# ROBOT-WSC/RGC-SLAM

Measured on AMD Instinct MI355X. Metric: registered scans/sec (16-beam -> 1M-pt map), higher is better.
Workload: dtype f32 points and neighbour search, f64 covariances and solve

## Files before the change

rgc-slam_amd/csrc/rgc_api.hip:

```cpp
#include "rgc_ctx.h"

static std::mutex g_live_mutex;
static std::unordered_set<const rgc_ctx*> g_live;
static std::atomic<unsigned long long> g_next_uid{1};

namespace rgcapi {

constexpr int kMaxK = 32;
constexpr unsigned kDevEvent = hipEventDisableTiming | hipEventReleaseToDevice;

bool ctx_alive(const rgc_ctx* c) {
  std::lock_guard<std::mutex> lk(g_live_mutex);
  return g_live.count(c) != 0;
}

int fail(rgc_ctx* c, int code, const char* fmt, ...) {
  if (c) {
    va_list ap;
    va_start(ap, fmt);
    vsnprintf(c->err, sizeof(c->err), fmt, ap);
    va_end(ap);
  }
  return code;
}
// ... 24 lines not shown
  memset(&at, 0, sizeof(at));
  if (hipPointerGetAttributes(&at, p) != hipSuccess) {
    (void)hipGetLastError();
    return fail(c, RGC_ERR_INVALID, "%s: %p is not memory the HIP runtime knows (a host pointer passed as a device pointer?)", what, p);
  }
  if (at.type != hipMemoryTypeDevice) return fail(c, RGC_ERR_INVALID, "%s: %p is not device memory", what, p);
  if (at.device != c->device) return fail(c, RGC_ERR_INVALID, "%s: %p lives on device %d, the context on device %d", what, p, at.device, c->device);
  void* base = nullptr;
  size_t size = 0;
  if (hipMemGetAddressRange((hipDeviceptr_t*)&base, &size, (hipDeviceptr_t)const_cast<void*>(p)) != hipSuccess) { (void)hipGetLastError(); return RGC_OK; }
  const size_t off = (size_t)((const char*)p - (const char*)base);
  if (off + bytes > size) return fail(c, RGC_ERR_INVALID, "%s: %zu bytes asked of an allocation that has %zu behind %p", what, bytes, size - off, p);
  return RGC_OK;
}

static void release(DevBuf& b) {
  if (b.p && !b.borrowed) (void)hipFree(b.p);
  b.p = nullptr;
  b.cap = 0;
  b.borrowed = false;
}

static void release_cloud(Cloud& cl) {
  for (DevBuf* b : {&cl.in_copy, &cl.cell_of, &cl.slot_of, &cl.cnt, &cl.start, &cl.block_sums, &cl.order_tmp, &cl.P, &cl.nx, &cl.ny, &cl.nz, &cl.segs,
                    &cl.cell_voxel, &cl.vox, &cl.vox_cell, &cl.need, &cl.qlist, &cl.cell_list, &cl.seed, &cl.nbr, &cl.rank_of, &cl.pos_of, &cl.qrank,
                    &cl.map_copy, &cl.todo, &cl.cache_small, &cl.c6})
    release(*b);
}

namespace {
struct ProfScope {
  rgc_ctx* c;
  bool on;
  ProfRegion r{};
  hipStream_t st;
  ProfScope(rgc_ctx* ctx, int kind, long long points, hipStream_t stream = nullptr) : c(ctx), on(ctx->prof_on && ((ctx->prof_mask >> kind) & 1u)), st(stream ? stream : ctx->stream) {
    if (!on) return;
    auto get = [&](hipEvent_t* e) {
      if (!c->ev_pool.empty()) { *e = c->ev_pool.back(); c->ev_pool.pop_back(); return true; }
      return hipEventCreate(e) == hipSuccess;
    };
    if (!get(&r.a)) { on = false; return; }
// ... 245 lines not shown
        if ((rc = ensure(c, cl.cnt, sizeof(int) * wc1 + 256))) return rc;
        if ((rc = ensure(c, cl.start, sizeof(int) * wc1))) return rc;
        if ((rc = ensure(c, cl.block_sums, sizeof(long long) * (wc1 / 2048 + 2)))) return rc;
        if (is_target && (rc = ensure(c, cl.cell_voxel, sizeof(int) * (size_t)w.ncell))) return rc;
        if (is_target) {
          const size_t vw = (size_t)(n < w.ncell ? n : w.ncell);
          if ((rc = ensure(c, cl.vox, sizeof(double) * rgck::kVoxRec * vw))) return rc;
          if ((rc = ensure(c, cl.vox_cell, sizeof(int) * vw))) return rc;
        }
      }
    }
    cl.grid = g;
    const size_t nc1 = (size_t)g.ncell + 1;
    const size_t ntot = nc1;
    int rc;
    if ((rc = ensure(c, cl.cell_of, sizeof(int) * n))) return rc;
    if ((rc = ensure(c, cl.slot_of, sizeof(int) * n))) return rc;
    size_t want_cells = ntot;
    if (hint && hint->reach_xy > 0) {
      const double e = hint->reach_xy / res + 6.0, ez = hint->reach_z / res + 6.0;
      const double cells = e * e * ez * 1.05;
      if (cells < 2.0e9 && cells <= (double)c->prm.max_cells && (size_t)cells > want_cells) want_cells = (size_t)cells;
    }
    if ((rc = ensure(c, cl.cnt, sizeof(int) * std::max(ntot, want_cells) + 256))) return rc;
    if ((rc = ensure(c, cl.start, sizeof(int) * std::max(nc1, want_cells)))) return rc;
    if ((rc = ensure(c, cl.block_sums, sizeof(long long) * (std::max(ntot, want_cells) / 2048 + 2)))) return rc;
    if ((rc = ensure(c, cl.order_tmp, sizeof(long long) * n))) return rc;
    if ((rc = ensure(c, cl.P, sizeof(float4) * ((size_t)n + 4)))) return rc;
    if ((rc = ensure(c, cl.segs, rgck::deferred_bytes(n)))) return rc;
    if ((rc = ensure(c, cl.nx, sizeof(double) * n))) return rc;
    if ((rc = ensure(c, cl.ny, sizeof(double) * n))) return rc;
    if ((rc = ensure(c, cl.nz, sizeof(double) * n))) return rc;
    if (is_target && (rc = ensure(c, cl.cell_voxel, sizeof(int) * std::max((size_t)g.ncell, want_cells)))) return rc;
    if (cl.cnt.p != cl.cnt_seen) { cl.cnt_clean = 0; cl.cnt_seen = cl.cnt.p; }
    if (cl.cnt_clean < ntot) {
      const size_t fill = std::min(cl.cnt.cap, (sizeof(int) * ntot + 255) & ~(size_t)255);
      HIPCHK(c, hipMemsetAsync(cl.cnt.p, 0, fill, s));
      cl.cnt_clean = fill / sizeof(int);
    }
    rgck::count_cells(s, cl.in, cl.stride_f, n, g, (int*)cl.cell_of.p, (int*)cl.slot_of.p, (int*)cl.cnt.p, hi, spec ? dsm + 6 : nullptr,
                      fuse_reframe ? &cl.rf : nullptr);
    rgck::scan_cells(s, (int*)cl.cnt.p, (int*)cl.start.p, (int)ntot, cl.block_sums.p, is_target ? (int*)cl.cell_voxel.p : nullptr,
                     is_target ? c->d_small + 7 : nullptr, hi, is_target ? nullptr : (float*)(c->d_small + 23));
    const bool with_cache = is_target && &cl == &c->tgt && cl.cache_on;
    const rgck::KnnSeeds sd = cloud_seeds(cl, is_target);
    rgck::place(s, n, (const int*)cl.cell_of.p, (const int*)cl.slot_of.p, (const int*)cl.start.p, (unsigned long long*)cl.order_tmp.p, hi,
                with_cache ? &sd.cache : nullptr);
    rgck::rank_gather(s, cl.in, cl.stride_f, n, (const int*)cl.cell_of.p, (const int*)cl.start.p, (const unsigned long long*)cl.order_tmp.p,
                      (float4*)cl.P.p, (int*)cl.segs.p, hi, with_cache ? &sd.cache : nullptr);
  }
  cl.lazy = 0;
  if (is_target && &cl == &c->tgt && c->lazy_margin > 0 && !c->lm_host && !general_route(c) && map_wide_r_of(c, cl) == 0) {
    int rc;
    const size_t vmax = (size_t)(n < cl.grid.ncell ? n : cl.grid.ncell);
    if ((rc = ensure(c, cl.vox, sizeof(double) * rgck::kVoxRec * vmax))) return rc;
    if ((rc = ensure(c, cl.vox_cell, sizeof(int) * vmax))) return rc;
    cl.lazy = 1;
    cl.nvox = -1;
    HIPCHK(c, hipGetLastError());
    HIPCHK(c, hipEventRecord(c->tgt_prepared, s));
    cl.ready = true;
    return RGC_OK;
  }
  cl.prepared_recorded = false;
// ... 299 lines not shown

int check_target_owner(rgc_ctx* c) {
  if (!c->tgt_owner) return RGC_OK;
  bool alive;
  unsigned long long owner_gen = 0;
  {
    std::lock_guard<std::mutex> lk(g_live_mutex);
    alive = g_live.count(c->tgt_owner) != 0 && c->tgt_owner->uid == c->tgt_owner_uid;
    if (alive) owner_gen = c->tgt_owner->tgt_generation;
  }
  if (!alive) {
    c->tgt_owner = nullptr;
    for (DevBuf* b : {&c->tgt.in_copy, &c->tgt.cell_of, &c->tgt.slot_of, &c->tgt.cnt, &c->tgt.start, &c->tgt.block_sums, &c->tgt.order_tmp, &c->tgt.P,
                      &c->tgt.nx, &c->tgt.ny, &c->tgt.nz, &c->tgt.segs, &c->tgt.cell_voxel, &c->tgt.vox, &c->tgt.vox_cell, &c->tgt.c6})
      release(*b);
    c->tgt.ready = false;
    c->tgt.n = 0;
    return fail(c, RGC_ERR_NO_INPUT, "the context whose target this one shared has been destroyed");
  }
  if (owner_gen != c->tgt_owner_gen)
    return fail(c, RGC_ERR_INVALID, "the shared target was rebuilt by its owner: rgc_share_target again");
  return RGC_OK;
}

static int validate_clouds(rgc_ctx* c, bool whole_target = true) {
  if (solve_in_flight(c)) return fail(c, RGC_ERR_INVALID, "a solve is in flight on this context: call rgc_align_end first");
  { int rc = check_target_owner(c); if (rc) return rc; }
  if ((c->tgt.ready && c->tgt.spec_used) || (c->src.ready && c->src.spec_used)) {
    HIPCHK(c, hipStreamSynchronize(c->stream2));
    HIPCHK(c, hipMemcpyAsync(c->h_small + 6, c->d_small + 6, sizeof(int), hipMemcpyDeviceToHost, c->stream));
// ... 160 lines not shown
  rgck::bbox(s, cl.in, cl.stride_f, n, cell, dsm, dsm + 6);
  HIPCHK(c, hipMemcpyAsync(hsm, dsm, words * sizeof(int), hipMemcpyDeviceToHost, s));
  HIPCHK(c, hipStreamSynchronize(s));
  if (hsm[6]) return fail(c, RGC_ERR_NONFINITE, "%s contains non-finite or absurd coordinates", name);
  int minc[3], dim[3];
  double ncell = 1.0;
  for (int a = 0; a < 3; a++) {
    minc[a] = hsm[a];
    dim[a] = hsm[3 + a] - hsm[a] + 1;
    ncell *= (double)dim[a];
  }
  if (ncell > (double)c->prm.max_cells || ncell > 2.0e9) return fail(c, RGC_ERR_GRID_TOO_LARGE, "%s exceeds max_cells", grid_name);
  const rgck::Grid g = rgck::make_grid(minc, dim, cell);
  cl.grid = g;
  const size_t nc1 = (size_t)g.ncell + 1;
  if ((rc = ensure(c, cl.cell_of, sizeof(int) * n))) return rc;
  if ((rc = ensure(c, cl.slot_of, sizeof(int) * n))) return rc;
  if ((rc = ensure(c, cl.cnt, sizeof(int) * nc1 + 256))) return rc;
  if ((rc = ensure(c, cl.start, sizeof(int) * nc1))) return rc;
  if (with_voxels && (rc = ensure(c, cl.cell_voxel, sizeof(int) * nc1))) return rc;
  if ((rc = ensure(c, cl.block_sums, sizeof(long long) * (nc1 / 2048 + 2)))) return rc;
  if ((rc = ensure(c, cl.order_tmp, sizeof(long long) * n))) return rc;
  if ((rc = ensure(c, cl.P, sizeof(float4) * ((size_t)n + 4)))) return rc;
  HIPCHK(c, hipMemsetAsync(cl.cnt.p, 0, (sizeof(int) * nc1 + 255) & ~(size_t)255, s));
  rgck::count_cells(s, cl.in, cl.stride_f, n, g, (int*)cl.cell_of.p, (int*)cl.slot_of.p, (int*)cl.cnt.p);
  rgck::scan_cells(s, (int*)cl.cnt.p, (int*)cl.start.p, (int)nc1, cl.block_sums.p, with_voxels ? (int*)cl.cell_voxel.p : nullptr, with_voxels ? dsm + 7 : nullptr);
  rgck::place(s, n, (const int*)cl.cell_of.p, (const int*)cl.slot_of.p, (const int*)cl.start.p, (unsigned long long*)cl.order_tmp.p);
  rgck::rank_gather(s, cl.in, cl.stride_f, n, (const int*)cl.cell_of.p, (const int*)cl.start.p, (const unsigned long long*)cl.order_tmp.p, (float4*)cl.P.p);
  return RGC_OK;
}

}

using namespace rgcapi;

extern "C" {

void rgc_default_params(rgc_params* p) {
  if (!p) return;
  p->voxel_res = 1.0;
  p->max_iterations = 25;
  p->lm_max_iterations = 10;
  p->rotation_eps = 2e-3;
// ... 188 lines not shown
  if ((rc = fetch_nvox(owner))) return fail(c, rc, "rgc_share_target: %s", owner->err);
  HIPCHK(c, hipStreamSynchronize(owner->stream2));
  HIPCHK(c, hipStreamSynchronize(owner->stream));
  HIPCHK(c, hipStreamSynchronize(c->stream2));
  HIPCHK(c, hipStreamSynchronize(c->stream));
  Cloud& d = c->tgt;
  const Cloud& o = owner->tgt;
  release_cloud(d);
  DevBuf* db[] = {&d.in_copy, &d.cell_of, &d.slot_of, &d.cnt, &d.start, &d.block_sums, &d.order_tmp, &d.P, &d.nx, &d.ny, &d.nz, &d.segs,
                  &d.cell_voxel, &d.vox, &d.vox_cell, &d.c6};
  const DevBuf* ob[] = {&o.in_copy, &o.cell_of, &o.slot_of, &o.cnt, &o.start, &o.block_sums, &o.order_tmp, &o.P, &o.nx, &o.ny, &o.nz, &o.segs,
                        &o.cell_voxel, &o.vox, &o.vox_cell, &o.c6};
  d.general = o.general;
  for (size_t k = 0; k < sizeof(db) / sizeof(db[0]); k++) { db[k]->p = ob[k]->p; db[k]->cap = ob[k]->cap; db[k]->borrowed = ob[k]->p != nullptr; }
  d.in = o.in; d.stride_f = o.stride_f; d.n = o.n; d.grid = o.grid; d.grid = o.grid; d.nvox = o.nvox; d.deferred_seen = o.deferred_seen;
  d.spec_ok = false; d.spec_used = false; d.cnt_clean = 0; d.cnt_seen = nullptr; d.lazy = 0;
  d.ready = true;
  const int small[2] = {0, o.nvox};
  HIPCHK(c, hipMemcpyAsync(c->d_small + 6, small, sizeof(small), hipMemcpyHostToDevice, c->stream));
  HIPCHK(c, hipStreamSynchronize(c->stream));
  c->tgt_owner = owner;
  c->tgt_owner_gen = owner->tgt_generation;
  c->tgt_owner_uid = owner->uid;
  c->map_bound = false;
  c->corr_valid = c->gicp_valid = false;
  c->deferred_known = false;
  c->main_has_target_prep = false;
  c->stats.n_target = o.n; c->stats.target_cells = o.grid.ncell; c->stats.n_voxels = o.nvox;
  return RGC_OK;
}

// ... 746 lines not shown
```

rgc-slam_amd/csrc/rgc_api_pre.hip:

```cpp
#include "rgc_ctx.h"

using namespace rgcapi;

int rgcapi::stage_in(rgc_ctx* c, const float* p, int n, int stride_bytes, int on_device, const float** d_in) {
  if (n > (1 << 27)) return fail(c, RGC_ERR_INVALID, "cloud has %d points, the limit is 2^27", n);
  if (on_device) {
    if (n > 0) { const int rk = check_device_range(c, p, (size_t)n * stride_bytes - (stride_bytes - 12), "input cloud"); if (rk) return rk; }
    *d_in = p;
    return RGC_OK;
  }
  const size_t bytes = (size_t)n * stride_bytes;
  int rc = ensure(c, c->pre_in, bytes);
  if (rc) return rc;
  HIPCHK(c, hipMemcpyAsync(c->pre_in.p, p, bytes, hipMemcpyHostToDevice, c->stream));
  *d_in = (const float*)c->pre_in.p;
  return RGC_OK;
}

extern "C" {

int rgc_deskew(rgc_ctx* c, float* xyzi, int n, int stride_bytes, const double q[4], const double t[3], int on_device) {
  if (!c || !xyzi || !q || !t || n < 0) return RGC_ERR_INVALID;
  if (stride_bytes < 16 || (stride_bytes & 3) || stride_bytes > 4096) return fail(c, RGC_ERR_INVALID, "de-skew needs x,y,z,intensity: stride_bytes >= 16");
  if (n == 0) return RGC_OK;
// ... 208 lines not shown
      seg_shift = 3;
      while (seg_shift < 30 && (double)(((long long)g.div[0] + (1ll << seg_shift) - 1) >> seg_shift) > nseg_max) seg_shift++;
    }
  }
  const size_t nr1 = (size_t)g.div[1] * (size_t)g.div[2] * (size_t)rgck::vg_segments(g, seg_shift) + 1;
  if ((rc = ensure(c, cl.cell_of, sizeof(int) * n))) return rc;
  if ((rc = ensure(c, cl.slot_of, sizeof(int) * n))) return rc;
  if ((rc = ensure(c, c->vg_pos, sizeof(int) * n))) return rc;
  if ((rc = ensure(c, c->vg_order, sizeof(int) * n))) return rc;
  if ((rc = ensure(c, c->vg_tmp, sizeof(long long) * n))) return rc;
  if ((rc = ensure(c, c->vg_leaf, sizeof(long long) * n))) return rc;
  if ((rc = ensure(c, cl.cnt, sizeof(int) * nr1))) return rc;
  if ((rc = ensure(c, cl.start, sizeof(int) * nr1))) return rc;
  const size_t row_bs = sizeof(long long) * (nr1 / 2048 + 2);
  if ((rc = ensure(c, cl.block_sums, row_bs + sizeof(int) * ((size_t)n / 2048 + 2)))) return rc;
  if (cl.cnt.p != cl.cnt_seen) { cl.cnt_clean = 0; cl.cnt_seen = cl.cnt.p; }
  if (cl.cnt_clean < nr1) {
    const size_t fill = std::min(cl.cnt.cap, (sizeof(int) * nr1 + 255) & ~(size_t)255);
    HIPCHK(c, hipMemsetAsync(cl.cnt.p, 0, fill, s));
  }
  cl.cnt_clean = std::max(cl.cnt_clean, nr1);
  if (!c->vg_flags_clean) HIPCHK(c, hipMemsetAsync(dsm + 6, 0, sizeof(int), s));
  c->vg_flags_clean = false;
  const bool packed = rgck::vg_rows(s, d_in, stride_f, n, inv, g, edge, seg_shift, (int*)cl.cell_of.p, (int*)cl.slot_of.p, (int*)c->vg_pos.p, (int*)cl.cnt.p,
                                    (int*)cl.start.p, cl.block_sums.p, (unsigned long long*)c->vg_tmp.p, (int*)c->vg_order.p, (unsigned long long*)c->vg_leaf.p,
                                    (int*)((char*)cl.block_sums.p + row_bs), d_out, dsm + 5);
  rt->chain = 1; rt->leaf_buckets = dense ? 1 : 0; rt->seg_shift = seg_shift; rt->nseg = rgck::vg_segments(g, seg_shift); rt->packed = packed ? 1 : 0;
  rt->edge = edge; rt->flags = 0;
  for (int a = 0; a < 3; a++) { rt->minb[a] = g.minb[a]; rt->div[a] = g.div[a]; }
  if (h_result) {
// ... 383 lines not shown
```

rgc-slam_amd/csrc/rgc_ctx.h:

```cpp
#pragma once
#include "../../include/rgc_hip.h"

#include <hip/hip_runtime.h>

#include <cfloat>
#include <climits>
#include <cmath>
#include <cstdarg>
#include <cstdint>
#include <cstdio>
#include <cstdlib>
#include <cstring>
#include <atomic>
#include <chrono>
#include <mutex>
#include <new>
#include <unordered_map>
#include <unordered_set>
#include <vector>

#include "rgc_kernels.h"

namespace rgcapi {

// ... 49 lines not shown
  bool ready = false;
  bool covs_user = false;
  DevBuf in_copy, cell_of, slot_of, cnt, start, block_sums, order_tmp, P, nx, ny, nz;
  DevBuf c6;
  bool general = false;
  DevBuf segs;
  int deferred_seen = -1;
  rgck::Grid grid{};
  rgck::Grid spec_grid{};
  bool spec_ok = false;
  bool spec_used = false;
  bool reframe_pending = false;
  rgck::Reframe rf{};
  size_t cnt_clean = 0;
  const void* cnt_seen = nullptr;
  DevBuf cell_voxel, vox, vox_cell;
  int nvox = -1;
  int lazy = 0;
  DevBuf need, qlist, cell_list;
  int need_stamp = 0;
  const void* need_seen = nullptr;
  int lazy_nq_seen = -1, lazy_ncell_seen = -1;
  DevBuf seed;
  const void* seed_key = nullptr;
  int seed_n = 0;
  bool seed_on = false;
  bool seed_warm = false;
  float seed_slack = 0.f;
  DevBuf nbr, rank_of, pos_of, qrank, map_copy, todo, cache_small;
  bool cache_on = false;
// ... 174 lines not shown
    if (_e != hipSuccess) {                                                                                \
      (void)hipGetLastError();              \
      return rgcapi::fail((c), RGC_ERR_HIP, "%s failed: %s (%s:%d)", #expr, hipGetErrorString(_e), __FILE__, __LINE__);               \
    }                                                                                                      \
  } while (0)

int fail(rgc_ctx* c, int code, const char* fmt, ...);
int ensure(rgc_ctx* c, DevBuf& b, size_t bytes);
int check_device_range(rgc_ctx* c, const void* p, size_t bytes, const char* what);
bool ctx_alive(const rgc_ctx* c);
const rgc_ctx::BoxHint* find_hint(const rgc_ctx* c, const void* p, int n);
void put_hint(rgc_ctx* c, const void* p, int n, const double lo[3], const double hi[3], double reach_xy = 0, double reach_z = 0);
void hint_from_leaf_grid(rgc_ctx* c, const float* out , int n_out, const rgck::LeafGrid& g, float leaf);
bool map_prep_finished(rgc_ctx* c);
int set_cloud(rgc_ctx* c, Cloud& cl, bool is_target, const float* xyz, int n, int stride_bytes, bool on_device, const rgck::Reframe* rf = nullptr);
int build_measured_grid(rgc_ctx* c, Cloud& cl, double cell, int* dsm, int* hsm, bool with_voxels, const char* name, const char* grid_name);
rgck::Pose pose_from(const double T[16]);
rgck::PoseF posef_from(const float T[16]);
int check_target_owner(rgc_ctx* c);
int need_inputs(rgc_ctx* c, bool validate = true);
int do_fitness(rgc_ctx* c, const float T[16], double* out);
void unpack_system(const double sums[28], double H[36], double b[6]);

inline bool solve_in_flight(const rgc_ctx* c) { return c->pend.active || c->gen_res.on; }
inline bool stride_ok(int stride_bytes) { return stride_bytes >= 12 && !(stride_bytes & 3) && stride_bytes <= 4096; }
template <class T>
inline bool pose12_finite(const T* m) {
  for (int i = 0; i < 12; i++)
    if (!std::isfinite(m[i])) return false;
  return true;
// ... 30 lines not shown
```

rgc-slam_amd/csrc/rgc_kernels.h:

```cpp
#pragma once
#include <hip/hip_runtime.h>

#include <cmath>

namespace rgck {

struct Grid {
  int minc[3];
  int dim[3];
  double res;
  int ncell;
  double inv_res;
};
inline double grid_inv_res(double res) {
  int e;
  return std::frexp(res, &e) == 0.5 ? 1.0 / res : 0.0;
}
inline Grid make_grid(const int minc[3], const int dim[3], double res) {
  Grid g{};
  double nc = 1.0;
  for (int a = 0; a < 3; a++) { g.minc[a] = minc[a]; g.dim[a] = dim[a]; nc *= (double)dim[a]; }
  g.res = res;
  g.inv_res = grid_inv_res(res);
  g.ncell = nc <= 2.0e9 ? (int)nc : -1;
// ... 38 lines not shown
  double fit_sum;
  int nvox, def_t, def_s, pad;
  int gen, cmd, mode, cur;
  float src_sq; int pad2;
  int lazy_nq, lazy_ncell;
};
struct LmInit { double x0[16], rot_eps, trans_eps, init_factor; int max_outer, max_inner; };
struct LmEarly { double x0[16]; int pad, pad2, outer, gen; };
struct FeParams { int n_scans; double min_range, max_range; };
struct LeafGrid { int minb[3]; int div[3]; };

constexpr int kAccum = 28;
constexpr int kVoxRec = 10;

void bbox(hipStream_t s, const float* in, int stride_f, int n, double res, int* mm6, int* flags, int hi = 0);
void count_cells(hipStream_t s, const float* in, int stride_f, int n, Grid g, int* cell_of, int* slot_of, int* cnt, int hi = 0, int* guard = nullptr,
                 const Reframe* rf = nullptr);
void scan_cells(hipStream_t s, int* cnt, int* start, int n, void* block_sums, int* cell_voxel, int* nvox, int hi = 0,
                float* sum_sq = nullptr );
void place(hipStream_t s, int n, const int* cell_of, const int* slot_of, const int* start, unsigned long long* order_tmp, int hi = 0,
           const KnnCache* cache = nullptr );
void exclusive_scan(hipStream_t s, const int* in, int* out, int n, int* block_sums , int hi = 0);
void rank_gather(hipStream_t s, const float* in, int stride_f, int n, const int* cell_of, const int* start,
                 const unsigned long long* order_tmp, float4* P, int* zero_me = nullptr, int hi = 0, const KnnCache* cache = nullptr);
size_t deferred_bytes(int n);
struct KnnSeeds {
  float* seed = nullptr;
  float slack = 0.f;
  bool warm = false;
  KnnCache cache;
};
bool knn_seeds_apply(int n, int k);
void knn_bulk(hipStream_t s, bool is_target, const float4* P, const int* start, Grid g, int n, int k, const void* deferred, double* nx,
              double* ny, double* nz, const int* guard = nullptr, int wide_r = 0,
              hipEvent_t ev0 = nullptr, hipEvent_t ev1 = nullptr ,
              const int* qlist = nullptr, const int* nq = nullptr, int q_est = 0, const KnnSeeds& seeds = KnnSeeds{},
              int stream_coop_waves = 0);
constexpr int kDeferredSlotEmptyByte = 0x80;
void footprint(hipStream_t s, const float* in, int stride_f, int n, Pose T, Grid g, int* need, int stamp, int margin, const float4* P, int n_map,
// ... 118 lines not shown
```

rgc-slam_amd/csrc/rgc_kernels.hip:

```cpp
#include "rgc_kernels.h"
#include "rgc_nn.h"
#include "rgc_lm.h"
#include <hip/hip_ext.h>

#include <limits.h>
#include <stddef.h>

#include <type_traits>

namespace rgck {

constexpr int WAVE = 64;

__device__ __forceinline__ int voxel_coord1(float x, double res) { return (int)floor((double)x / res - 0.5); }

__device__ __forceinline__ int wave_min(int v) {
#pragma unroll
  for (int o = 32; o > 0; o >>= 1) v = min(v, __shfl_xor(v, o));
  return v;
}
__device__ __forceinline__ int wave_max(int v) {
#pragma unroll
  for (int o = 32; o > 0; o >>= 1) v = max(v, __shfl_xor(v, o));
  return v;
// ... 128 lines not shown
}

__device__ __forceinline__ constexpr int row_dy(int r, int D, int R) { return r % D - R; }
__device__ __forceinline__ constexpr int row_dz(int r, int D, int R) { return r / D - R; }

__device__ __forceinline__ float4 reframe_point(const Reframe& rf, int i) {
  const float* p = rf.src + (size_t)i * rf.src_stride_f;
  const Quat& q = rf.q;
  const double vx = (double)p[0], vy = (double)p[1], vz = (double)p[2];
  double ux = q.y * vz - q.z * vy, uy = q.z * vx - q.x * vz, uz = q.x * vy - q.y * vx;
  ux += ux; uy += uy; uz += uz;
  return make_float4((float)(vx + q.w * ux + (q.y * uz - q.z * uy) + rf.t[0]), (float)(vy + q.w * uy + (q.z * ux - q.x * uz) + rf.t[1]),
                     (float)(vz + q.w * uz + (q.x * uy - q.y * ux) + rf.t[2]), rf.src_stride_f > 3 ? p[3] : 0.f);
}

template <bool kReframe>
__global__ void k_count(const float* __restrict__ in, int stride_f, int n, Grid g, int* __restrict__ cell_of, int* __restrict__ slot_of,
                        int* cnt, int* guard, int prio, Reframe rf) {
  wave_prio(prio);
  const int i = blockIdx.x * blockDim.x + threadIdx.x;
  const bool valid = i < n;
  const int lane = threadIdx.x & (WAVE - 1);
  int c = -1 - lane;
#ifdef RGC_LAB_TURN
  if (kReframe && i == 0) {
    const unsigned long long now = wall_clock64(), post = atomicExch(&g_lab_turn[3], 0ull);
    if (post) { atomicAdd(&g_lab_turn[0], now - post); atomicAdd(&g_lab_turn[1], 1ull); atomicMax(&g_lab_turn[2], now - post); }
  }
#endif
  if (valid) {
    float pt[3];
    if (kReframe) {
      if (rf.copy) {
// ... 16 lines not shown
    int cx, cy, cz;
    if (guard) {
      const float x = p[0], y = p[1], z = p[2];
      const bool fin = fabsf(x) <= 1.0e8f && fabsf(y) <= 1.0e8f && fabsf(z) <= 1.0e8f;
      cx = fin ? cell_coord(x, g) - g.minc[0] : 0;
      cy = fin ? cell_coord(y, g) - g.minc[1] : 0;
      cz = fin ? cell_coord(z, g) - g.minc[2] : 0;
      const bool inside = cx >= 0 && cx < g.dim[0] && cy >= 0 && cy < g.dim[1] && cz >= 0 && cz < g.dim[2];
      if (!fin || !inside) { atomicOr(guard, fin ? 2 : 1); cx = cy = cz = 0; }
    } else {
      cx = cell_coord(p[0], g) - g.minc[0];
      cy = cell_coord(p[1], g) - g.minc[1];
      cz = cell_coord(p[2], g) - g.minc[2];
    }
    c = cell_index(g, cx, cy, cz);
    cell_of[i] = c;
  }
  unsigned long long todo = __ballot(valid);
  int lead = lane, rank = 0, group = 1;
  while (todo) {
    const int l0 = __ffsll((long long)todo) - 1;
    const int cl = __shfl(c, l0);
    const unsigned long long same = __ballot(valid && c == cl);
    if (valid && c == cl) {
      lead = l0;
      rank = __popcll(same & ((1ull << lane) - 1ull));
      group = __popcll(same);
    }
    todo &= ~same;
  }
  int base = 0;
  if (valid && lane == lead) base = atomicAdd(&cnt[c], group);
  base = __shfl(base, lead);
  if (valid) slot_of[i] = base + rank;
}

constexpr int SCAN_T = 256, SCAN_V = 8, SCAN_B = SCAN_T * SCAN_V;

__device__ __forceinline__ int block_exclusive_scan(int v, int* total) {
  __shared__ int wsum[SCAN_T / WAVE];
  int lane = threadIdx.x & (WAVE - 1), w = threadIdx.x / WAVE;
  int inc = v;
#pragma unroll
  for (int o = 1; o < WAVE; o <<= 1) {
    int t = __shfl_up(inc, o);
    if (lane >= o) inc += t;
  }
  if (lane == WAVE - 1) wsum[w] = inc;
  __syncthreads();
  int base = 0, tot = 0;
#pragma unroll
  for (int j = 0; j < SCAN_T / WAVE; j++) {
// ... 197 lines not shown
#pragma unroll
  for (int j = 0; j < SCAN_V; j++) {
    const int i = base + j;
    if (i < n) {
      start[i] = (int)(unsigned)ex;
      if (cell_voxel && i < n - 1) cell_voxel[i] = v[j] > 0 ? (int)(ex >> 32) : -1;
    }
    ex += scan_value(v[j]);
  }
}

constexpr int kOrdIdxBits = 27, kOrdCntBits = 18;
constexpr unsigned long long kOrdIdxMask = (1ull << kOrdIdxBits) - 1ull;
constexpr int kOrdCntMax = (1 << kOrdCntBits) - 1;
__device__ __forceinline__ bool cache_redo(const KnnCache& kc) { return *kc.epoch == kc.frame || kc.overflow[(kc.frame - 1) & 1] == kc.frame - 1; }
__global__ void k_place(int n, const int* __restrict__ cell_of, const int* __restrict__ slot_of, const int* __restrict__ start,
                        unsigned long long* __restrict__ order_tmp, int prio, KnnCache kc) {
  wave_prio(prio);
  const int i = blockIdx.x * blockDim.x + threadIdx.x;
  if (kc.nbr && i < kTodoLists && cache_redo(kc)) kc.todo_cnt[i] = 0;
  if (i >= n) return;
  const int c = cell_of[i], slot = slot_of[i];
  const int s0 = start[c], cnt = start[c + 1] - s0;
  const bool big = cnt > kOrdCntMax;
  order_tmp[s0 + slot] = (unsigned long long)(unsigned)i | ((unsigned long long)(big ? 0 : slot) << kOrdIdxBits) |
                         ((unsigned long long)(big ? 0 : cnt) << (kOrdIdxBits + kOrdCntBits));
}

__global__ void k_rank_gather(const float* __restrict__ in, int stride_f, int n, const int* __restrict__ cell_of,
                              const int* __restrict__ start, const unsigned long long* __restrict__ order_tmp, float4* __restrict__ P, int* zero_me,
                              int prio, KnnCache kc) {
  wave_prio(prio);
  int s = blockIdx.x * blockDim.x + threadIdx.x;
  if (s == 0 && zero_me) { zero_me[0] = 0; zero_me[1] = 0; zero_me[2] = 0; }
  if (s < 4) P[n + s] = make_float4(1.0e30f, 1.0e30f, 1.0e30f, __int_as_float(-1));
  if (s >= n) return;
  const unsigned long long rec = order_tmp[s];
  const int i = (int)(rec & kOrdIdxMask);
  const bool ranked = kc.nbr && !cache_redo(kc);
  int my_rank = 0;
  if (ranked) my_rank = kc.rank_of[i];
  const int cnt = (int)(rec >> (kOrdIdxBits + kOrdCntBits)) & kOrdCntMax;
  int s0, s1;
  if (cnt > 0) {
    s0 = s - ((int)(rec >> kOrdIdxBits) & kOrdCntMax);
    s1 = s0 + cnt;
  } else {
    const int c = cell_of[i];
    s0 = start[c];
    s1 = start[c + 1];
  }
  const float* p = in + (size_t)i * stride_f;
  const float px = p[0], py = p[1], pz = p[2];
  const unsigned* lo = reinterpret_cast<const unsigned*>(order_tmp);
  constexpr unsigned kLoMask = (unsigned)kOrdIdxMask;
  int rank = 0;
  int t = s0;
  for (; t + 8 <= s1; t += 8) {
    unsigned o[8];
#pragma unroll
    for (int u = 0; u < 8; u++) o[u] = lo[2 * (size_t)(t + u)];
#pragma unroll
    for (int u = 0; u < 8; u++) rank += ((int)(o[u] & kLoMask) < i);
// ... 3007 lines not shown
                  int want_H, double* partials, double* out56) {
  MapregPose ps[2];
  for (int b = 0; b < 2; b++) {
    const double* q = x14 + 7 * b;
    ps[b] = MapregPose{feat[2 * b], fac[2 * b], nfeat[2 * b], feat[2 * b + 1], fac[2 * b + 1], nfeat[2 * b + 1], Quat{q[0], q[1], q[2], q[3]},
                       {q[4], q[5], q[6]}};
  }
  const int nb = max(max(mapreg_blocks(nfeat[0], nfeat[1]), mapreg_blocks(nfeat[2], nfeat[3])), 1);
  hipLaunchKernelGGL(k_mapreg_terms, dim3(nb, 2), dim3(LIN_T), 0, s, ps[0], ps[1], huber_a, want_H, partials);
  hipLaunchKernelGGL(k_mapreg_fold, dim3(2 * kAccum), dim3(WAVE), 0, s, partials, nb, out56);
}

void bbox(hipStream_t s, const float* in, int stride_f, int n, double res, int* mm6, int* flags, int hi) {
  hipLaunchKernelGGL(k_bbox, dim3(min(nblk(n, 256), 1024)), dim3(256), 0, s, in, stride_f, n, res, mm6, flags, hi);
}
void count_cells(hipStream_t s, const float* in, int stride_f, int n, Grid g, int* cell_of, int* slot_of, int* cnt, int hi, int* guard,
                 const Reframe* rf) {
  if (rf) hipLaunchKernelGGL(k_count<true>, dim3(nblk(n, kGridT)), dim3(kGridT), 0, s, in, 4, n, g, cell_of, slot_of, cnt, guard, hi, *rf);
  else hipLaunchKernelGGL(k_count<false>, dim3(nblk(n, kGridT)), dim3(kGridT), 0, s, in, stride_f, n, g, cell_of, slot_of, cnt, guard, hi, Reframe{});
}
void scan_cells(hipStream_t s, int* cnt, int* start, int n, void* block_sums, int* cell_voxel, int* nvox, int hi, float* sum_sq) {
  const int nb = nblk(n, SCAN_B);
  unsigned long long* bs = (unsigned long long*)block_sums;
  if (nb > 1 || sum_sq) hipLaunchKernelGGL(k_cells_reduce, dim3(nb), dim3(SCAN_T), 0, s, cnt, n, bs, hi, sum_sq);
  if (nb <= 4096) {
    hipLaunchKernelGGL(k_cells_scan_write<true>, dim3(nb), dim3(SCAN_T), 0, s, cnt, start, n, bs, nb, cell_voxel, nvox, hi);
  } else {
    hipLaunchKernelGGL(k_cells_scan_sums, dim3(1), dim3(SCAN_T), 0, s, bs, nb, nvox, hi);
    hipLaunchKernelGGL(k_cells_scan_write<false>, dim3(nb), dim3(SCAN_T), 0, s, cnt, start, n, bs, nb, cell_voxel, nvox, hi);
  }
}
void place(hipStream_t s, int n, const int* cell_of, const int* slot_of, const int* start, unsigned long long* order_tmp, int hi, const KnnCache* cache) {
  hipLaunchKernelGGL(k_place, dim3(nblk(n, kGridT)), dim3(kGridT), 0, s, n, cell_of, slot_of, start, order_tmp, hi, cache ? *cache : KnnCache{});
}
void exclusive_scan(hipStream_t s, const int* in, int* out, int n, int* block_sums, int hi) {
  const int nb = nblk(n, SCAN_B);
  hipLaunchKernelGGL(k_scan_block, dim3(nb), dim3(SCAN_T), 0, s, in, out, n, block_sums, hi);
  if (nb > 1) {
    hipLaunchKernelGGL(k_scan_sums, dim3(1), dim3(SCAN_T), 0, s, block_sums, nb, hi);
    hipLaunchKernelGGL(k_scan_add, dim3(nb), dim3(SCAN_T), 0, s, out, n, block_sums, hi);
  }
}
void rank_gather(hipStream_t s, const float* in, int stride_f, int n, const int* cell_of, const int* start,
                 const unsigned long long* order_tmp, float4* P, int* zero_me, int hi, const KnnCache* cache) {
  hipLaunchKernelGGL(k_rank_gather, dim3(nblk(n, kGridT)), dim3(kGridT), 0, s, in, stride_f, n, cell_of, start, order_tmp, P, zero_me, hi,
                     cache ? *cache : KnnCache{});
}
size_t deferred_bytes(int n) { return sizeof(int) * (2 * (size_t)n + 16); }

static Deferred deferred_of(const void* buf, int n) {
  int* base = (int*)const_cast<void*>(buf);
  return Deferred{base + 16, (float*)(base + 16 + (size_t)n), base, nullptr, nullptr, nullptr, nullptr, 0.f, KnnCache{}, 0,
                  0, base + 1, reinterpret_cast<unsigned long long*>(base + 16), 0};
}

template <int KC, bool kExact>
static void knn_bulk_kc(hipStream_t s, bool is_target, const float4* P, const int* start, Grid g, int n, int k, const void* deferred,
                        double* nx, double* ny, double* nz, const int* guard, int wide_r, hipEvent_t ev0, hipEvent_t ev1,
                        const int* qlist, const int* nq, int q_est, const KnnSeeds& seeds, int stream_coop_waves) {
  Deferred df = deferred_of(deferred, n);
  df.guard = guard;
// ... 188 lines not shown
```

Before: 2744.

## Fuse per-block cell totals into count kernel and pack cell/slot as int2

```diff
diff --git a/rgc-slam_amd/csrc/rgc_api.hip b/rgc-slam_amd/csrc/rgc_api.hip
--- a/rgc-slam_amd/csrc/rgc_api.hip
+++ b/rgc-slam_amd/csrc/rgc_api.hip
@@ -62,6 +62,17 @@
   return RGC_OK;
 }
 
+int ensure_block_sums(rgc_ctx* c, Cloud& cl, size_t bytes, hipStream_t s) {
+  int rc;
+  if ((rc = ensure(c, cl.block_sums, bytes))) return rc;
+  if (cl.block_sums.p != cl.bs_seen || cl.block_sums.cap != cl.bs_cap) {
+    HIPCHK(c, hipMemsetAsync(cl.block_sums.p, 0, cl.block_sums.cap, s));
+    cl.bs_seen = cl.block_sums.p;
+    cl.bs_cap = cl.block_sums.cap;
+  }
+  return RGC_OK;
+}
+
 static void release(DevBuf& b) {
   if (b.p && !b.borrowed) (void)hipFree(b.p);
   b.p = nullptr;
@@ -74,6 +85,7 @@
                     &cl.cell_voxel, &cl.vox, &cl.vox_cell, &cl.need, &cl.qlist, &cl.cell_list, &cl.seed, &cl.nbr, &cl.rank_of, &cl.pos_of, &cl.qrank,
                     &cl.map_copy, &cl.todo, &cl.cache_small, &cl.c6})
     release(*b);
+  cl.bs_seen = nullptr;
 }
 
 namespace {
@@ -349,8 +361,7 @@
     const size_t nc1 = (size_t)g.ncell + 1;
     const size_t ntot = nc1;
     int rc;
-    if ((rc = ensure(c, cl.cell_of, sizeof(int) * n))) return rc;
-    if ((rc = ensure(c, cl.slot_of, sizeof(int) * n))) return rc;
+    if ((rc = ensure(c, cl.cell_of, sizeof(int2) * n))) return rc;
     size_t want_cells = ntot;
     if (hint && hint->reach_xy > 0) {
       const double e = hint->reach_xy / res + 6.0, ez = hint->reach_z / res + 6.0;
@@ -359,7 +370,7 @@
     }
     if ((rc = ensure(c, cl.cnt, sizeof(int) * std::max(ntot, want_cells) + 256))) return rc;
     if ((rc = ensure(c, cl.start, sizeof(int) * std::max(nc1, want_cells)))) return rc;
-    if ((rc = ensure(c, cl.block_sums, sizeof(long long) * (std::max(ntot, want_cells) / 2048 + 2)))) return rc;
+    if ((rc = ensure_block_sums(c, cl, sizeof(long long) * (std::max(ntot, want_cells) / 2048 + 2), s))) return rc;
     if ((rc = ensure(c, cl.order_tmp, sizeof(long long) * n))) return rc;
     if ((rc = ensure(c, cl.P, sizeof(float4) * ((size_t)n + 4)))) return rc;
     if ((rc = ensure(c, cl.segs, rgck::deferred_bytes(n)))) return rc;
@@ -373,16 +384,15 @@
       HIPCHK(c, hipMemsetAsync(cl.cnt.p, 0, fill, s));
       cl.cnt_clean = fill / sizeof(int);
     }
-    rgck::count_cells(s, cl.in, cl.stride_f, n, g, (int*)cl.cell_of.p, (int*)cl.slot_of.p, (int*)cl.cnt.p, hi, spec ? dsm + 6 : nullptr,
-                      fuse_reframe ? &cl.rf : nullptr);
+    rgck::count_cells(s, cl.in, cl.stride_f, n, g, (int2*)cl.cell_of.p, (int*)cl.cnt.p, is_target ? cl.block_sums.p : nullptr, hi,
+                      spec ? dsm + 6 : nullptr, fuse_reframe ? &cl.rf : nullptr);
     rgck::scan_cells(s, (int*)cl.cnt.p, (int*)cl.start.p, (int)ntot, cl.block_sums.p, is_target ? (int*)cl.cell_voxel.p : nullptr,
-                     is_target ? c->d_small + 7 : nullptr, hi, is_target ? nullptr : (float*)(c->d_small + 23));
+                     is_target ? c->d_small + 7 : nullptr, hi, is_target ? nullptr : (float*)(c->d_small + 23), is_target);
     const bool with_cache = is_target && &cl == &c->tgt && cl.cache_on;
     const rgck::KnnSeeds sd = cloud_seeds(cl, is_target);
-    rgck::place(s, n, (const int*)cl.cell_of.p, (const int*)cl.slot_of.p, (const int*)cl.start.p, (unsigned long long*)cl.order_tmp.p, hi,
-                with_cache ? &sd.cache : nullptr);
-    rgck::rank_gather(s, cl.in, cl.stride_f, n, (const int*)cl.cell_of.p, (const int*)cl.start.p, (const unsigned long long*)cl.order_tmp.p,
-                      (float4*)cl.P.p, (int*)cl.segs.p, hi, with_cache ? &sd.cache : nullptr);
+    rgck::place(s, n, (const int2*)cl.cell_of.p, (const int*)cl.start.p, (unsigned long long*)cl.order_tmp.p, hi, with_cache ? &sd.cache : nullptr);
+    rgck::rank_gather(s, cl.in, cl.stride_f, n, (const int2*)cl.cell_of.p, (const int*)cl.start.p, (const unsigned long long*)cl.order_tmp.p,
+                      (float4*)cl.P.p, cl.block_sums.p, (int)ntot, (int*)cl.segs.p, hi, with_cache ? &sd.cache : nullptr);
   }
   cl.lazy = 0;
   if (is_target && &cl == &c->tgt && c->lazy_margin > 0 && !c->lm_host && !general_route(c) && map_wide_r_of(c, cl) == 0) {
@@ -712,6 +722,7 @@
     for (DevBuf* b : {&c->tgt.in_copy, &c->tgt.cell_of, &c->tgt.slot_of, &c->tgt.cnt, &c->tgt.start, &c->tgt.block_sums, &c->tgt.order_tmp, &c->tgt.P,
                       &c->tgt.nx, &c->tgt.ny, &c->tgt.nz, &c->tgt.segs, &c->tgt.cell_voxel, &c->tgt.vox, &c->tgt.vox_cell, &c->tgt.c6})
       release(*b);
+    c->tgt.bs_seen = nullptr;
     c->tgt.ready = false;
     c->tgt.n = 0;
     return fail(c, RGC_ERR_NO_INPUT, "the context whose target this one shared has been destroyed");
@@ -902,19 +913,20 @@
   const rgck::Grid g = rgck::make_grid(minc, dim, cell);
   cl.grid = g;
   const size_t nc1 = (size_t)g.ncell + 1;
-  if ((rc = ensure(c, cl.cell_of, sizeof(int) * n))) return rc;
-  if ((rc = ensure(c, cl.slot_of, sizeof(int) * n))) return rc;
+  if ((rc = ensure(c, cl.cell_of, sizeof(int2) * n))) return rc;
   if ((rc = ensure(c, cl.cnt, sizeof(int) * nc1 + 256))) return rc;
   if ((rc = ensure(c, cl.start, sizeof(int) * nc1))) return rc;
   if (with_voxels && (rc = ensure(c, cl.cell_voxel, sizeof(int) * nc1))) return rc;
-  if ((rc = ensure(c, cl.block_sums, sizeof(long long) * (nc1 / 2048 + 2)))) return rc;
+  if ((rc = ensure_block_sums(c, cl, sizeof(long long) * (nc1 / 2048 + 2), s))) return rc;
   if ((rc = ensure(c, cl.order_tmp, sizeof(long long) * n))) return rc;
   if ((rc = ensure(c, cl.P, sizeof(float4) * ((size_t)n + 4)))) return rc;
   HIPCHK(c, hipMemsetAsync(cl.cnt.p, 0, (sizeof(int) * nc1 + 255) & ~(size_t)255, s));
-  rgck::count_cells(s, cl.in, cl.stride_f, n, g, (int*)cl.cell_of.p, (int*)cl.slot_of.p, (int*)cl.cnt.p);
-  rgck::scan_cells(s, (int*)cl.cnt.p, (int*)cl.start.p, (int)nc1, cl.block_sums.p, with_voxels ? (int*)cl.cell_voxel.p : nullptr, with_voxels ? dsm + 7 : nullptr);
-  rgck::place(s, n, (const int*)cl.cell_of.p, (const int*)cl.slot_of.p, (const int*)cl.start.p, (unsigned long long*)cl.order_tmp.p);
-  rgck::rank_gather(s, cl.in, cl.stride_f, n, (const int*)cl.cell_of.p, (const int*)cl.start.p, (const unsigned long long*)cl.order_tmp.p, (float4*)cl.P.p);
+  rgck::count_cells(s, cl.in, cl.stride_f, n, g, (int2*)cl.cell_of.p, (int*)cl.cnt.p, cl.block_sums.p);
+  rgck::scan_cells(s, (int*)cl.cnt.p, (int*)cl.start.p, (int)nc1, cl.block_sums.p, with_voxels ? (int*)cl.cell_voxel.p : nullptr, with_voxels ? dsm + 7 : nullptr,
+                   0, nullptr, true);
+  rgck::place(s, n, (const int2*)cl.cell_of.p, (const int*)cl.start.p, (unsigned long long*)cl.order_tmp.p);
+  rgck::rank_gather(s, cl.in, cl.stride_f, n, (const int2*)cl.cell_of.p, (const int*)cl.start.p, (const unsigned long long*)cl.order_tmp.p, (float4*)cl.P.p,
+                    cl.block_sums.p, (int)nc1);
   return RGC_OK;
 }
 
@@ -1133,7 +1145,7 @@
   d.general = o.general;
   for (size_t k = 0; k < sizeof(db) / sizeof(db[0]); k++) { db[k]->p = ob[k]->p; db[k]->cap = ob[k]->cap; db[k]->borrowed = ob[k]->p != nullptr; }
   d.in = o.in; d.stride_f = o.stride_f; d.n = o.n; d.grid = o.grid; d.grid = o.grid; d.nvox = o.nvox; d.deferred_seen = o.deferred_seen;
-  d.spec_ok = false; d.spec_used = false; d.cnt_clean = 0; d.cnt_seen = nullptr; d.lazy = 0;
+  d.spec_ok = false; d.spec_used = false; d.cnt_clean = 0; d.cnt_seen = nullptr; d.bs_seen = nullptr; d.lazy = 0;
   d.ready = true;
   const int small[2] = {0, o.nvox};
   HIPCHK(c, hipMemcpyAsync(c->d_small + 6, small, sizeof(small), hipMemcpyHostToDevice, c->stream));
diff --git a/rgc-slam_amd/csrc/rgc_api_pre.hip b/rgc-slam_amd/csrc/rgc_api_pre.hip
--- a/rgc-slam_amd/csrc/rgc_api_pre.hip
+++ b/rgc-slam_amd/csrc/rgc_api_pre.hip
@@ -246,6 +246,7 @@
   if ((rc = ensure(c, cl.start, sizeof(int) * nr1))) return rc;
   const size_t row_bs = sizeof(long long) * (nr1 / 2048 + 2);
   if ((rc = ensure(c, cl.block_sums, row_bs + sizeof(int) * ((size_t)n / 2048 + 2)))) return rc;
+  cl.bs_seen = nullptr;
   if (cl.cnt.p != cl.cnt_seen) { cl.cnt_clean = 0; cl.cnt_seen = cl.cnt.p; }
   if (cl.cnt_clean < nr1) {
     const size_t fill = std::min(cl.cnt.cap, (sizeof(int) * nr1 + 255) & ~(size_t)255);
diff --git a/rgc-slam_amd/csrc/rgc_ctx.h b/rgc-slam_amd/csrc/rgc_ctx.h
--- a/rgc-slam_amd/csrc/rgc_ctx.h
+++ b/rgc-slam_amd/csrc/rgc_ctx.h
@@ -87,6 +87,8 @@
   rgck::Reframe rf{};
   size_t cnt_clean = 0;
   const void* cnt_seen = nullptr;
+  const void* bs_seen = nullptr;
+  size_t bs_cap = 0;
   DevBuf cell_voxel, vox, vox_cell;
   int nvox = -1;
   int lazy = 0;
@@ -291,6 +293,7 @@
 void hint_from_leaf_grid(rgc_ctx* c, const float* out , int n_out, const rgck::LeafGrid& g, float leaf);
 bool map_prep_finished(rgc_ctx* c);
 int set_cloud(rgc_ctx* c, Cloud& cl, bool is_target, const float* xyz, int n, int stride_bytes, bool on_device, const rgck::Reframe* rf = nullptr);
+int ensure_block_sums(rgc_ctx* c, Cloud& cl, size_t bytes, hipStream_t s);
 int build_measured_grid(rgc_ctx* c, Cloud& cl, double cell, int* dsm, int* hsm, bool with_voxels, const char* name, const char* grid_name);
 rgck::Pose pose_from(const double T[16]);
 rgck::PoseF posef_from(const float T[16]);
diff --git a/rgc-slam_amd/csrc/rgc_kernels.h b/rgc-slam_amd/csrc/rgc_kernels.h
--- a/rgc-slam_amd/csrc/rgc_kernels.h
+++ b/rgc-slam_amd/csrc/rgc_kernels.h
@@ -76,15 +76,16 @@
 constexpr int kVoxRec = 10;
 
 void bbox(hipStream_t s, const float* in, int stride_f, int n, double res, int* mm6, int* flags, int hi = 0);
-void count_cells(hipStream_t s, const float* in, int stride_f, int n, Grid g, int* cell_of, int* slot_of, int* cnt, int hi = 0, int* guard = nullptr,
-                 const Reframe* rf = nullptr);
+void count_cells(hipStream_t s, const float* in, int stride_f, int n, Grid g, int2* cell_slot, int* cnt, void* block_sums, int hi = 0,
+                 int* guard = nullptr, const Reframe* rf = nullptr);
 void scan_cells(hipStream_t s, int* cnt, int* start, int n, void* block_sums, int* cell_voxel, int* nvox, int hi = 0,
-                float* sum_sq = nullptr );
-void place(hipStream_t s, int n, const int* cell_of, const int* slot_of, const int* start, unsigned long long* order_tmp, int hi = 0,
+                float* sum_sq = nullptr , bool totals_ready = false);
+void place(hipStream_t s, int n, const int2* cell_slot, const int* start, unsigned long long* order_tmp, int hi = 0,
            const KnnCache* cache = nullptr );
 void exclusive_scan(hipStream_t s, const int* in, int* out, int n, int* block_sums , int hi = 0);
-void rank_gather(hipStream_t s, const float* in, int stride_f, int n, const int* cell_of, const int* start,
-                 const unsigned long long* order_tmp, float4* P, int* zero_me = nullptr, int hi = 0, const KnnCache* cache = nullptr);
+void rank_gather(hipStream_t s, const float* in, int stride_f, int n, const int2* cell_slot, const int* start,
+                 const unsigned long long* order_tmp, float4* P, void* block_sums, int cells1, int* zero_me = nullptr, int hi = 0,
+                 const KnnCache* cache = nullptr);
 size_t deferred_bytes(int n);
 struct KnnSeeds {
   float* seed = nullptr;
diff --git a/rgc-slam_amd/csrc/rgc_kernels.hip b/rgc-slam_amd/csrc/rgc_kernels.hip
--- a/rgc-slam_amd/csrc/rgc_kernels.hip
+++ b/rgc-slam_amd/csrc/rgc_kernels.hip
@@ -166,9 +166,12 @@
                      (float)(vz + q.w * uz + (q.x * uy - q.y * ux) + rf.t[2]), rf.src_stride_f > 3 ? p[3] : 0.f);
 }
 
+constexpr int SCAN_T = 256, SCAN_V = 8, SCAN_B = SCAN_T * SCAN_V, SCAN_SHIFT = 11;
+static_assert(SCAN_B == 1 << SCAN_SHIFT, "k_count names a cell's scan block by a shift");
+
 template <bool kReframe>
-__global__ void k_count(const float* __restrict__ in, int stride_f, int n, Grid g, int* __restrict__ cell_of, int* __restrict__ slot_of,
-                        int* cnt, int* guard, int prio, Reframe rf) {
+__global__ void k_count(const float* __restrict__ in, int stride_f, int n, Grid g, int2* __restrict__ cell_slot, int* cnt,
+                        unsigned long long* block_sums, int* guard, int prio, Reframe rf) {
   wave_prio(prio);
   const int i = blockIdx.x * blockDim.x + threadIdx.x;
   const bool valid = i < n;
@@ -215,7 +218,6 @@
       cz = cell_coord(p[2], g) - g.minc[2];
     }
     c = cell_index(g, cx, cy, cz);
-    cell_of[i] = c;
   }
   unsigned long long todo = __ballot(valid);
   int lead = lane, rank = 0, group = 1;
@@ -232,11 +234,21 @@
   }
   int base = 0;
   if (valid && lane == lead) base = atomicAdd(&cnt[c], group);
+  if (block_sums) {
+    const bool first = valid && lane == lead && base == 0;
+    const int b = c >> SCAN_SHIFT;
+    todo = __ballot(valid);
+    while (todo) {
+      const int l0 = __ffsll((long long)todo) - 1;
+      const int bl = __shfl(b, l0);
+      const unsigned long long same = __ballot(valid && b == bl), fresh = __ballot(first && b == bl);
+      if (lane == l0) atomicAdd(&block_sums[bl], (unsigned long long)__popcll(same) | ((unsigned long long)__popcll(fresh) << 32));
+      todo &= ~same;
+    }
+  }
   base = __shfl(base, lead);
-  if (valid) slot_of[i] = base + rank;
-}
-
-constexpr int SCAN_T = 256, SCAN_V = 8, SCAN_B = SCAN_T * SCAN_V;
+  if (valid) cell_slot[i] = make_int2(c, base + rank);
+}
 
 __device__ __forceinline__ int block_exclusive_scan(int v, int* total) {
   __shared__ int wsum[SCAN_T / WAVE];
@@ -464,24 +476,26 @@
 constexpr unsigned long long kOrdIdxMask = (1ull << kOrdIdxBits) - 1ull;
 constexpr int kOrdCntMax = (1 << kOrdCntBits) - 1;
 __device__ __forceinline__ bool cache_redo(const KnnCache& kc) { return *kc.epoch == kc.frame || kc.overflow[(kc.frame - 1) & 1] == kc.frame - 1; }
-__global__ void k_place(int n, const int* __restrict__ cell_of, const int* __restrict__ slot_of, const int* __restrict__ start,
+__global__ void k_place(int n, const int2* __restrict__ cell_slot, const int* __restrict__ start,
                         unsigned long long* __restrict__ order_tmp, int prio, KnnCache kc) {
   wave_prio(prio);
   const int i = blockIdx.x * blockDim.x + threadIdx.x;
   if (kc.nbr && i < kTodoLists && cache_redo(kc)) kc.todo_cnt[i] = 0;
   if (i >= n) return;
-  const int c = cell_of[i], slot = slot_of[i];
+  const int2 cs = cell_slot[i];
+  const int c = cs.x, slot = cs.y;
   const int s0 = start[c], cnt = start[c + 1] - s0;
   const bool big = cnt > kOrdCntMax;
   order_tmp[s0 + slot] = (unsigned long long)(unsigned)i | ((unsigned long long)(big ? 0 : slot) << kOrdIdxBits) |
                          ((unsigned long long)(big ? 0 : cnt) << (kOrdIdxBits + kOrdCntBits));
 }
 
-__global__ void k_rank_gather(const float* __restrict__ in, int stride_f, int n, const int* __restrict__ cell_of,
+__global__ void k_rank_gather(const float* __restrict__ in, int stride_f, int n, const int2* __restrict__ cell_slot,
                               const int* __restrict__ start, const unsigned long long* __restrict__ order_tmp, float4* __restrict__ P, int* zero_me,
-                              int prio, KnnCache kc) {
+                              unsigned long long* block_sums, int nb, int prio, KnnCache kc) {
   wave_prio(prio);
   int s = blockIdx.x * blockDim.x + threadIdx.x;
+  for (int j = s; j < nb; j += (int)(gridDim.x * blockDim.x)) block_sums[j] = 0ull;
   if (s == 0 && zero_me) { zero_me[0] = 0; zero_me[1] = 0; zero_me[2] = 0; }
   if (s < 4) P[n + s] = make_float4(1.0e30f, 1.0e30f, 1.0e30f, __int_as_float(-1));
   if (s >= n) return;
@@ -496,7 +510,7 @@
     s0 = s - ((int)(rec >> kOrdIdxBits) & kOrdCntMax);
     s1 = s0 + cnt;
   } else {
-    const int c = cell_of[i];
+    const int c = cell_slot[i].x;
     s0 = start[c];
     s1 = start[c + 1];
   }
@@ -3534,15 +3548,16 @@
 void bbox(hipStream_t s, const float* in, int stride_f, int n, double res, int* mm6, int* flags, int hi) {
   hipLaunchKernelGGL(k_bbox, dim3(min(nblk(n, 256), 1024)), dim3(256), 0, s, in, stride_f, n, res, mm6, flags, hi);
 }
-void count_cells(hipStream_t s, const float* in, int stride_f, int n, Grid g, int* cell_of, int* slot_of, int* cnt, int hi, int* guard,
+void count_cells(hipStream_t s, const float* in, int stride_f, int n, Grid g, int2* cell_slot, int* cnt, void* block_sums, int hi, int* guard,
                  const Reframe* rf) {
-  if (rf) hipLaunchKernelGGL(k_count<true>, dim3(nblk(n, kGridT)), dim3(kGridT), 0, s, in, 4, n, g, cell_of, slot_of, cnt, guard, hi, *rf);
-  else hipLaunchKernelGGL(k_count<false>, dim3(nblk(n, kGridT)), dim3(kGridT), 0, s, in, stride_f, n, g, cell_of, slot_of, cnt, guard, hi, Reframe{});
-}
-void scan_cells(hipStream_t s, int* cnt, int* start, int n, void* block_sums, int* cell_voxel, int* nvox, int hi, float* sum_sq) {
+  unsigned long long* bs = (unsigned long long*)block_sums;
+  if (rf) hipLaunchKernelGGL(k_count<true>, dim3(nblk(n, kGridT)), dim3(kGridT), 0, s, in, 4, n, g, cell_slot, cnt, bs, guard, hi, *rf);
+  else hipLaunchKernelGGL(k_count<false>, dim3(nblk(n, kGridT)), dim3(kGridT), 0, s, in, stride_f, n, g, cell_slot, cnt, bs, guard, hi, Reframe{});
+}
+void scan_cells(hipStream_t s, int* cnt, int* start, int n, void* block_sums, int* cell_voxel, int* nvox, int hi, float* sum_sq, bool totals_ready) {
   const int nb = nblk(n, SCAN_B);
   unsigned long long* bs = (unsigned long long*)block_sums;
-  if (nb > 1 || sum_sq) hipLaunchKernelGGL(k_cells_reduce, dim3(nb), dim3(SCAN_T), 0, s, cnt, n, bs, hi, sum_sq);
+  if ((nb > 1 && !totals_ready) || sum_sq) hipLaunchKernelGGL(k_cells_reduce, dim3(nb), dim3(SCAN_T), 0, s, cnt, n, bs, hi, sum_sq);
   if (nb <= 4096) {
     hipLaunchKernelGGL(k_cells_scan_write<true>, dim3(nb), dim3(SCAN_T), 0, s, cnt, start, n, bs, nb, cell_voxel, nvox, hi);
   } else {
@@ -3550,8 +3565,8 @@
     hipLaunchKernelGGL(k_cells_scan_write<false>, dim3(nb), dim3(SCAN_T), 0, s, cnt, start, n, bs, nb, cell_voxel, nvox, hi);
   }
 }
-void place(hipStream_t s, int n, const int* cell_of, const int* slot_of, const int* start, unsigned long long* order_tmp, int hi, const KnnCache* cache) {
-  hipLaunchKernelGGL(k_place, dim3(nblk(n, kGridT)), dim3(kGridT), 0, s, n, cell_of, slot_of, start, order_tmp, hi, cache ? *cache : KnnCache{});
+void place(hipStream_t s, int n, const int2* cell_slot, const int* start, unsigned long long* order_tmp, int hi, const KnnCache* cache) {
+  hipLaunchKernelGGL(k_place, dim3(nblk(n, kGridT)), dim3(kGridT), 0, s, n, cell_slot, start, order_tmp, hi, cache ? *cache : KnnCache{});
 }
 void exclusive_scan(hipStream_t s, const int* in, int* out, int n, int* block_sums, int hi) {
   const int nb = nblk(n, SCAN_B);
@@ -3561,10 +3576,10 @@
     hipLaunchKernelGGL(k_scan_add, dim3(nb), dim3(SCAN_T), 0, s, out, n, block_sums, hi);
   }
 }
-void rank_gather(hipStream_t s, const float* in, int stride_f, int n, const int* cell_of, const int* start,
-                 const unsigned long long* order_tmp, float4* P, int* zero_me, int hi, const KnnCache* cache) {
-  hipLaunchKernelGGL(k_rank_gather, dim3(nblk(n, kGridT)), dim3(kGridT), 0, s, in, stride_f, n, cell_of, start, order_tmp, P, zero_me, hi,
-                     cache ? *cache : KnnCache{});
+void rank_gather(hipStream_t s, const float* in, int stride_f, int n, const int2* cell_slot, const int* start,
+                 const unsigned long long* order_tmp, float4* P, void* block_sums, int cells1, int* zero_me, int hi, const KnnCache* cache) {
+  hipLaunchKernelGGL(k_rank_gather, dim3(nblk(n, kGridT)), dim3(kGridT), 0, s, in, stride_f, n, cell_slot, start, order_tmp, P, zero_me,
+                     (unsigned long long*)block_sums, block_sums ? nblk(cells1, SCAN_B) : 0, hi, cache ? *cache : KnnCache{});
 }
 size_t deferred_bytes(int n) { return sizeof(int) * (2 * (size_t)n + 16); }
 
```

Result: slower. 2385 (-13.1%).
